# rnpnr/ogl_beamforming

Measured on AMD Instinct MI355X. Metric: beamformed voxels/s (and %HBM-roofline), 256-ch 3D DAS 512^3, 1/2/4/8 GPUs, higher is better.
Workload: dtype f32

## Files before the change

### ogl_beamforming_amd/csrc/bf_kernels.h

```cpp
#ifndef BF_KERNELS_H
#define BF_KERNELS_H

#include <stdint.h>
#include <hip/hip_runtime_api.h>

static const int bf_kind_byte_size[6]     = {2, 4, 4, 8, 2, 4};
static const int bf_kind_element_size[6]  = {2, 2, 4, 4, 2, 2};
static const int bf_kind_element_count[6] = {1, 2, 1, 2, 1, 2};
static const int bf_kind_complex[6]       = {0, 1, 0, 1, 0, 1};
enum { BF_BASE_I16 = 0, BF_BASE_F32 = 1, BF_BASE_F16 = 2 };
static const int bf_kind_base[6] = {BF_BASE_I16, BF_BASE_I16, BF_BASE_F32, BF_BASE_F32, BF_BASE_F16, BF_BASE_F16};

typedef struct {
	float    sin_a, cos_a;
	float    focus_x, focus_z;
	uint32_t flags;
	float    pad[3];
} BfTransmit;
enum {
	BF_TX_ROWS    = 1u << 0,
	BF_RX_ROWS    = 1u << 1,
	BF_TX_NONE    = 1u << 2,
	BF_TX_PLANE   = 1u << 3,
	BF_RX_COLUMNS = 1u << 4,
};

enum { BF_DAS_RCA = 0, BF_DAS_HERCULES = 1, BF_DAS_FORCES = 2, BF_DAS_READI = 3 };

typedef struct {
	float xdc_transform[16];
	float voxel_transform[16];
	float pitch[2];
	const void       *rf;
	void             *out;
	const BfTransmit *transmits;
	const int16_t    *sparse_elements;
	const uint16_t   *readi_hadamard;
	unsigned long long *pair_counter;
	uint32_t *tile_counters;
	int32_t  family, interpolation, complex_data, coherency_weighting;
	int32_t  acquisition_count, channel_count, sample_count, sparse;
	float    sampling_frequency, inv_sampling_frequency, demodulation_frequency;
	float    inv_speed_of_sound, time_offset, f_number;
	float    speed_of_sound;
	float    turns_per_sample;
	float    first_transmit_weight;
	uint32_t size[3];
	uint32_t z_first, z_count;
	uint32_t readi_group_count, readi_group;
	uint32_t tile_shift[3];
	uint32_t split_shift;
	uint32_t blocks[3];
	uint32_t depth_major;
	uint32_t band_rows;
	uint32_t zero_offset;
	uint32_t tile_window_shift;
	float    edge_margin;
	uint32_t row_ends;
} BfDasArgs;

#define BF_STAGED_PAIRED_GROUP_MAX 60u

typedef struct {
	uint32_t u_axis;
	uint32_t u_shift, v_shift;
	uint32_t threads;
	uint32_t channel_chunk;
	uint32_t lds_bytes;
	uint32_t tiles[3];
	uint32_t depth_major;
	uint32_t walk_columns;
	uint32_t window_shift;
	uint32_t zero_offset;
	uint32_t uniform;
	uint32_t window_samples;
	uint32_t table_stride;
	void    *tables;
	uint32_t *violations;
} BfSeparableArgs;

typedef struct {
	float   *table;
	float   *extremes;
	uint32_t table_pitch;
	uint32_t inner_count, outer_count;
	uint32_t inner_coord;
	uint32_t inner_is_transmit;
	uint32_t tiles[3];
	uint32_t rows;
	uint32_t depth_major;
	uint32_t band_rows;
	uint32_t zero_offset;
	float    unit_scale2, samples_per_unit;
	void    *pairs;
	uint32_t phase_local;
} BfHerculesArgs;

typedef struct {
	const void *raw; void *out;
	const int16_t *channel_mapping;
	uint64_t in_row_bytes, out_row_bytes;
	uint32_t channels;
	int32_t  a1s2, base;
	uint32_t a1s2_scalars;
} BfIngestArgs;

typedef struct {
	const void *left, *right; void *out;
	uint32_t size[3];
	int64_t  in_stride[3], out_stride[3];
	int32_t  in_kind, out_kind, interleave;
} BfReshapeArgs;

typedef struct {
	const void *in; void *out;
	const float *hadamard_t;
	const float *hadamard_base;
	uint32_t     hadamard_base_order;
	uint32_t transmit_count, channel_count, sample_count;
	int64_t  out_stride[3];
	int32_t  in_kind, out_kind;
} BfDecodeArgs;

typedef struct {
	const void *in; void *out;
	const float *coefficients;
	const float *phasors;
	uint32_t filter_length, decimation, sample_count, batch_sample_count;
	int32_t  complex_filter, demodulate;
	float    sampling_frequency, demodulation_frequency;
	int64_t  in_stride[3], out_stride[3];
	int64_t  in_elements;
	uint32_t channels, transmits;
	int32_t  in_kind, out_kind;
} BfFilterArgs;

static inline uint32_t bf_walk_columns(uint32_t tiles_u) { return tiles_u % 4u == 0 ? 4u : (tiles_u % 2u == 0 ? 2u : 1u); }
#ifdef __HIPCC__
static __device__ __forceinline__ void bf_column_walk(uint32_t tile, uint32_t tiles_u, uint32_t tiles_z, uint32_t g, uint32_t &tu, uint32_t &tv, uint32_t &zl)
{
	const uint32_t r = tile / g, col = r / tiles_z, per_row = tiles_u / g;
	zl = r % tiles_z;
	tu = (col % per_row) * g + tile % g;
	tv = col / per_row;
// ... 58 lines not shown
```

### ogl_beamforming_amd/csrc/das_select.cpp

```cpp
#include "das_select.h"
#include "host_math.h"
#include "../../include/ogl_beamformer_lib.h"
#include <cmath>
#include <cstdio>
#include <cstdlib>
#include <cstring>

namespace bf {

const char *das_path_name(int path)
{
	static const char *names[] = {"general kernel", "separable-delay gather kernel", "separable-delay LDS-staged kernel", "per-voxel factored kernel",
	                              "HERCULES aligned-grid kernel", "per-voxel factored kernel with block-wide LDS staging",
	                              "?", "none: the frame is cleared"};
	return path >= 0 && path <= 7 ? names[path] : "?";
}

const char *das_kernel_name(int path)
{
	static const char *names[] = {"das_kernel", "das_rca_separable_kernel", "das_rca_staged_kernel", "das_factored_kernel",
	                              "das_hercules_kernel", "das_tile_kernel", "?", "(none)"};
	return path >= 0 && path <= 7 ? names[path] : "?";
}

// ... 242 lines not shown
	q.tiles[0] = (nu + (1u << best_u) - 1) >> best_u;
	q.tiles[1] = (nv + (1u << best_v) - 1) >> best_v;
	q.tiles[2] = zcount;
	q.walk_columns = 1u;
	return true;
}

static bool plan_staged(const BfDasArgs &a, const std::vector<BfTransmit> &tx, const float *xdc, const float *vox,
                        uint32_t zcount, BfSeparableArgs &q, bool allow_uniform = true)
{
	const Hooks &hk = hooks();
	const bool cplx = a.complex_data != 0;
	const bool cubic = a.interpolation == 2;
	if (a.interpolation != 1 && !(cubic && cplx)) return false;
	const uint32_t C = (uint32_t)a.channel_count, A = (uint32_t)a.acquisition_count;
	if ((uint64_t)C * A * (uint64_t)a.sample_count * (cplx ? 8u : 4u) >= (1ull << 31)) return false;
	const uint32_t A4 = (A + 3u) & ~3u;
	const int u_axis = (int)q.u_axis, v_axis = 1 - u_axis;
	const int r = (tx[0].flags & BF_RX_ROWS) ? 1 : 0, w = (tx[0].flags & BF_TX_ROWS) ? 1 : 0;
	float m[16];
	m4_mul(xdc, vox, m);
	const float samples_per_metre = a.sampling_frequency * a.inv_speed_of_sound;
	float step_u = std::fabs(m[4 * u_axis + r]) / (float)(a.size[u_axis] > 1 ? a.size[u_axis] - 1 : 1) * samples_per_metre;
	float step_v = std::fabs(vox[4 * v_axis + w]) / (float)(a.size[v_axis] > 1 ? a.size[v_axis] - 1 : 1) * samples_per_metre;
	bool all_plane = true; float max_sin = 0.f;
	for (const BfTransmit &t : tx) {
		all_plane &= (t.flags & BF_TX_PLANE) != 0;
		max_sin = std::fmax(max_sin, std::fabs(t.sin_a));
	}
	if (tx[0].flags & BF_TX_NONE) step_v = 0.f;
	else if (all_plane)           step_v *= max_sin;

	const uint32_t lds_cu = 160u * 1024u;
	uint32_t best_waves = 0, best_score = 0;
	BfSeparableArgs best = q;
	for (uint32_t threads_shift = 10; threads_shift >= 9; threads_shift--) {
		for (uint32_t vs = 4; vs <= 6; vs++) {
			if (vs + 4 > threads_shift) continue;
			uint32_t us = threads_shift - vs;
			if (us > 6) continue;
			if ((u_axis == 0 ? us : vs) < 4) continue;
			float spread = step_u * (float)((1u << us) - 1) + step_v * (float)((1u << vs) - 1);
			if (!(spread >= 0.f && spread <= 60.f)) continue;
			uint32_t need = (uint32_t)std::ceil(spread * 1.001f) + (cubic ? 6 : 4);
			uint32_t ws = need <= 32 ? 5 : need <= 64 ? 6 : 0;
			if (!ws) continue;
			if (hk.staged_shape_set) {
				const unsigned fu = (unsigned)hk.staged_shape[0], fv = (unsigned)hk.staged_shape[1], fw = (unsigned)hk.staged_shape[2];
				if (fu != us || fv != vs) continue;
				if (fw < ws || fw > 6) continue;
				ws = fw;
			}
			const bool uniform = allow_uniform && cplx && !cubic && u_axis == 0 && threads_shift == 10 && us == 6 && vs == 4 &&
			                     !hk.staged_nouniform;
			const uint32_t window = 1u << ws;
			if (((uint64_t)A4 << ws) > ((uint64_t)(cplx ? 4 : 8) << threads_shift)) continue;
			const uint64_t stage_elements = (uint64_t)A4 * window;
			for (uint32_t chunk = 8; chunk <= 64; chunk *= 2) {
				uint32_t cc = chunk < C ? chunk : C;
				uint64_t lds = cubic ? 12ull * ((uint64_t)A4 << vs) + 16ull * ((uint64_t)cc << us) + 32ull * (stage_elements + 3) + 4ull * (A4 + cc + 1) + 128
				             : cplx ? (uniform ? 0ull : 12ull * ((uint64_t)A4 << vs)) + 16ull * ((uint64_t)cc << us) + 16ull * (stage_elements + 3) + 4ull * (A4 + cc + 1) + 128
				                    :  4ull * ((uint64_t)A4 << vs) +  8ull * ((uint64_t)cc << us) +  8ull * (stage_elements + 4) + 4ull * (A4 + cc + 1) + 128;
				lds = (lds + 15) & ~15ull;
				if (lds > lds_cu) continue;
				uint32_t blocks = (uint32_t)(lds_cu / lds), by_waves = (cubic ? 1024u : 2048u) >> threads_shift;
				if (blocks > by_waves) blocks = by_waves;
				uint32_t waves = blocks << (threads_shift - 6);
				uint32_t balance = us > vs ? us - vs : vs - us;
				uint32_t score = (blocks >= 2 ? 1000u : 0u) + (cc << 2) + (8 - balance) + (window == 32 ? 500u : 0u) +
				                 (uniform && window == 32 ? 2000u : 0u);
				if (waves > best_waves || (waves == best_waves && score > best_score)) {
					best_waves = waves; best_score = score;
					best.u_shift = us; best.v_shift = vs; best.threads = 1u << threads_shift;
					best.channel_chunk = cc; best.lds_bytes = (uint32_t)lds; best.window_shift = ws; best.window_samples = window;
					best.uniform = uniform ? 1u : 0u;
					best.table_stride = uniform ? 4u * A4 + 16u + 16u * (A4 / 4u) * 48u : 0u;
				}
				if (cc == C) break;
			}
		}
	}
	if (best_waves && allow_uniform && cplx && !cubic && !hk.staged_nouniform && best.threads == 1024 && best.u_shift == 5 && best.v_shift == 5 &&
	    best.window_samples == 32) {
		const uint32_t ngroups = (A4 + BF_STAGED_PAIRED_GROUP_MAX - 1u) / BF_STAGED_PAIRED_GROUP_MAX;
		const uint64_t group = ((A4 + ngroups - 1u) / ngroups + 3u) & ~3u;
		const uint32_t cc = best.channel_chunk;
		uint64_t lds = 16ull * (group * 64 + 3) + 16ull * ((uint64_t)((cc + 1) & ~1u) << 5) + 4ull * (A4 + cc + 1) + 128;
		lds = (lds + 15) & ~15ull;
		if (ngroups <= 2 && lds <= lds_cu / 2 && ((cc & 1u) == 0 || cc == C)) {
			best.uniform = 2u;
			best.lds_bytes = (uint32_t)lds;
			best.table_stride = 4u * A4 + 16u + 16u * (A4 / 2u) * 48u;
		}
	}
	if (hk.staged_checked) best.depth_major |= 2u;
	if (best.uniform && (best.depth_major & 1u)) best.depth_major |= 4u;
	if (hk.debug)
		std::fprintf(stderr, "[beamformer] staged plan: step_u %.3f step_v %.3f waves %u u %u v %u w %u chunk %u lds %u uniform %u\n",
		             step_u, step_v, best_waves, best.u_shift, best.v_shift, best.window_samples, best.channel_chunk, best.lds_bytes, best.uniform);
	if (!best_waves) return false;
	q = best;
	uint32_t nu = a.size[u_axis], nv = a.size[v_axis];
	q.tiles[0] = (nu + (1u << q.u_shift) - 1) >> q.u_shift;
	q.tiles[1] = (nv + (1u << q.v_shift) - 1) >> q.v_shift;
	q.tiles[2] = zcount;
	q.walk_columns = bf_walk_columns(q.tiles[0]);
	return true;
}

static const uint32_t kHerculesRows = 8u;

static bool plan_hercules(const BfDasArgs &a, const std::vector<BfTransmit> &tx, const float *xdc, const float *vox,
                          uint32_t zcount, bool forced, BfHerculesArgs &q)
{
	if (a.family != BF_DAS_HERCULES || tx.empty()) return false;
	if (!forced) {
		if (a.size[0] < 32 || a.split_shift) return false;
		if (((a.size[0] + 63u) & ~63u) > a.size[0] + a.size[0] / 3u) return false;
	}
	auto W = [&](int row, int col) { return vox[4 * col + row]; };
	auto X = [&](int row, int col) { return xdc[4 * col + row]; };
	auto moves = [&](int row, int col) {
		if (a.size[col] <= 1) return false;
		for (int k = 0; k < 3; k++) if (X(row, k) != 0.f && W(k, col) != 0.f) return true;
		return false;
	};
	int inner = -1;
	for (int coord = 0; coord < 2 && inner < 0; coord++)
		if (!moves(coord, 0) && !moves(coord, 2)) inner = coord;
	if (inner == 0 && !moves(1, 0) && !moves(1, 2) && !moves(0, 1) && moves(1, 1)) inner = 1;
	if (inner < 0) return false;
	const bool rx_cols = (tx[0].flags & BF_RX_COLUMNS) != 0;
	const int  tx_coord = rx_cols ? 1 : 0;
	const uint32_t A = (uint32_t)a.acquisition_count, C = (uint32_t)a.channel_count;
	const uint32_t transmits = A - (a.sparse ? 1u : 0u);
	if (!transmits || !C) return false;
	q.inner_coord       = (uint32_t)inner;
	q.inner_is_transmit = inner == tx_coord;
	q.inner_count       = q.inner_is_transmit ? transmits : C;
	q.outer_count       = q.inner_is_transmit ? C : transmits;
	q.table_pitch       = (q.inner_count + 8u + 3u) & ~3u;
	q.tiles[0] = (a.size[0] + 63u) / 64u;
	q.rows     = kHerculesRows;
	q.tiles[1] = (a.size[1] + q.rows - 1u) / q.rows;
	q.tiles[2] = zcount;
	{
		float m[16];
		m4_mul(xdc, vox, m);
		const uint32_t ext[3] = {a.size[0], a.size[1], zcount};
		int depth = 2; float best = -1.f;
		for (int i = 0; i < 3; i++) {
			if (ext[i] <= 1) continue;
			float step = std::fabs(m[4 * i + 2]) / (float)(a.size[i] > 1 ? a.size[i] - 1 : 1);
			if (step > best) { best = step; depth = i; }
		}
		q.depth_major = tile_walk(depth, zcount, q.tiles[1], q.band_rows);
	}
	{
		static float cached_fs = 0.f, cached_c = 0.f, cached_s2 = 1.f, cached_k = 0.f;
		if (cached_fs != a.sampling_frequency || cached_c != a.speed_of_sound) {
			const double k_exact = (double)a.sampling_frequency / (double)a.speed_of_sound;
			double best = 1e9;
			for (int i = -4096; i <= 4096; i++) {
				uint32_t bits = 0x3F800000u + (uint32_t)i;
				float s2; std::memcpy(&s2, &bits, sizeof s2);
				double s  = std::sqrt((double)s2);
				float  kk = (float)(k_exact / s);
				double err = std::fabs((double)kk * s / k_exact - 1.0);
				if (err < best) { best = err; cached_s2 = s2; cached_k = kk; }
			}
			cached_fs = a.sampling_frequency; cached_c = a.speed_of_sound;
		}
// ... 417 lines not shown
```

### ogl_beamforming_amd/csrc/das_staged.hip

```cpp
#include "das_common.h"

typedef int i32x2 __attribute__((ext_vector_type(2)));
typedef __attribute__((address_space(3))) f32x2 lds_f32x2;
typedef __attribute__((address_space(3))) f32x4 lds_f32x4;
typedef float f32x3 __attribute__((ext_vector_type(3)));
typedef __attribute__((address_space(3))) f32x3 lds_f32x3;

__device__ __forceinline__ float staged_phase_turns(float k, float index)
{
	float p = k * index;
	float e = __builtin_fmaf(k, index, -p);
	return hw_fract(p) + e;
}

__device__ __forceinline__ bool staged_tile_of(const BfSeparableArgs &q, bool global_tables, uint32_t &tu, uint32_t &tv, uint32_t &zl)
{
	const bool paired = global_tables && (q.depth_major & 4u);
	const uint32_t zchunks = (q.tiles[2] + 31u) >> 5;
	const uint32_t total = paired ? q.tiles[0] * q.tiles[1] * zchunks * 32u : q.tiles[0] * q.tiles[1] * q.tiles[2];
	const uint32_t per   = (total + 7u) / 8u;
	const uint32_t tile  = (blockIdx.x & 7u) * per + (blockIdx.x >> 3);
	if (tile >= total) return false;
	if (paired) {
		uint32_t r = tile >> 5;
// ... 253 lines not shown
				else return 0.f;
			};
			auto batches = [&](auto checked) {
				constexpr bool CHECK = decltype(checked)::value;
				uint32_t lane_id = tid;
				asm volatile("" : "+v"(lane_id));
				const uint32_t lane_v = u_axis == 0 ? lane_id >> q.u_shift : lane_id & (V - 1);
				uint32_t tcs_at = tcs_base + (lane_v << 4), tz_at = tz_base + (lane_v << 3);
				uint32_t m_bits = 0x4B000002u;
				[[maybe_unused]] bool window_left = false;
				const f32x2 rr = {r_rel, r_rel};
				const_f32x4 *uni_row = nullptr;
				if constexpr (UNI)
					uni_row = (const_f32x4 *)(uintptr_t)(tile_tab + 4u * (uint32_t)A4 + 16u +
					                                      (size_t)__builtin_amdgcn_readfirstlane((int)(tid >> 6)) * (size_t)(A4 / 4) * 48u);
				for (int a = 0; a < A4; a += 4, m_bits += 4u * W) {
					uint32_t at[4]; f32x4 tap[4];
					const float M = __builtin_bit_cast(float, m_bits);
					const f32x2 M2 = {M, M};
					f32x4 cs01, cs23; f32x2 tz01, tz23;
					if constexpr (UNI) {
						const f32x4 tz = uni_row[0];
						cs01 = uni_row[1]; cs23 = uni_row[2];
						tz01 = f32x2{tz.x, tz.y}; tz23 = f32x2{tz.z, tz.w};
						uni_row += 3;
					} else {
						cs01 = *(lds_f32x4 *)(uintptr_t)tcs_at;
						cs23 = *(lds_f32x4 *)(uintptr_t)(tcs_at + V * 16u);
						tz01 = *(lds_f32x2 *)(uintptr_t)tz_at;
						tz23 = *(lds_f32x2 *)(uintptr_t)(tz_at + V * 8u);
						tcs_at += 2u * V * 16u; tz_at += 2u * V * 8u;
					}
					const f32x2 p01 = rr + tz01, p23 = rr + tz23;
					const f32x2 y01 = p01 + M2,  y23 = p23 + M2;
					const float ys[4] = {y01.x, y01.y, y23.x, y23.y};
					#pragma unroll
					for (int k = 0; k < 4; k++) {
						const uint32_t yb = __builtin_bit_cast(uint32_t, ys[k]);
						asm("v_lshlrev_b16 %0, 4, %1" : "=v"(at[k]) : "v"(yb));
						if constexpr (CHECK) {
							uint32_t k_abs = (uint32_t)((int)(yb - m_bits) + rfloor[cl] + tfl[a + k]);
							at[k] = k_abs < ulast ? at[k] + (uint32_t)k * W * 16u : (stage_elements + 2u) * 16u;
							window_left |= __builtin_amdgcn_ballot_w64((yb - m_bits) > W - 2u) != 0ull;
						}
					}
					#pragma unroll
					for (int k = 0; k < 4; k++) tap[k] = *(lds_f32x4 *)(uintptr_t)(at[k] + (CHECK ? 0u : (uint32_t)k * W * 16u));
					const float q0 = term(f32x2{cs01.x, cs01.y}, p01.x, tap[0]);
					const float q1 = term(f32x2{cs01.z, cs01.w}, p01.y, tap[1]);
					const float q2 = term(f32x2{cs23.x, cs23.y}, p23.x, tap[2]);
					const float q3 = term(f32x2{cs23.z, cs23.w}, p23.y, tap[3]);
					if constexpr (CW) { mag2 += f32x2{q0, q1}; mag2 += f32x2{q2, q3}; }
				}
				if constexpr (CHECK) { if (window_left) staged_violation_raise(); }
			};
			if (wave_safe) batches(std::false_type{});
			else           batches(std::true_type{});
			float sum_x = acc1.x - acc2.y, sum_y = acc1.y + acc2.x;
			asm volatile("" : "+v"(sum_x), "+v"(sum_y));
			const f32x4 r = *(volatile lds_f32x4 *)(uintptr_t)((uint32_t)(uintptr_t)(lds_f32x4 *)Rl + (uint32_t)cl * U * 16u);
			coherent.x = __builtin_fmaf(sum_x, r.y, __builtin_fmaf(-sum_y, r.z, coherent.x));
			coherent.y = __builtin_fmaf(sum_x, r.z, __builtin_fmaf(sum_y, r.y, coherent.y));
			if constexpr (CW) incoherent = __builtin_fmaf(__builtin_fabsf(r.w), mag2.x + mag2.y, incoherent);
		}
	}
	if (q.depth_major & 2u) staged_violation_report(tid);
	if (!inside) return;

	uint32_t x, y, lane_u_unused, thread = tid;
	asm volatile("" : "+v"(thread));
	voxel_of(thread, x, y, lane_u_unused);
	uint64_t out_index = (uint64_t)p.size[0] * p.size[1] * zl + (uint64_t)p.size[0] * y + x;
	if constexpr (CW) coherent = coherent * (coherent / incoherent);
	reinterpret_cast<f32x2 *>(p.out)[out_index] = coherent;
}

template <bool CW, int NL>
__device__ __forceinline__ void staged_paired_body(const BfDasArgs &p, const BfSeparableArgs &q)
{
	extern __shared__ __attribute__((aligned(16))) f32x4 staged_lds[];
	constexpr uint32_t U = 32, W = 32, B = 2 * W;
	const int C = p.channel_count, A = p.acquisition_count, S = p.sample_count;
	const uint32_t A4 = ((uint32_t)A + 3u) & ~3u;
	const uint32_t ngroups = (A4 + BF_STAGED_PAIRED_GROUP_MAX - 1u) / BF_STAGED_PAIRED_GROUP_MAX;
	const uint32_t G0 = ((A4 + ngroups - 1u) / ngroups + 3u) & ~3u;
	const int chunk = (int)q.channel_chunk;
	f32x4 *stage  = staged_lds + 2;
	f32x4 *R      = stage + (size_t)G0 * B + 1;
	int   *tfl    = reinterpret_cast<int *>(R + (size_t)((chunk + 1) & ~1) * U);
	int   *rfloor = tfl + A4;

	uint32_t tu, tv, zl;
	if (!staged_tile_of(q, true, tu, tv, zl)) return;
	const uint32_t z = p.z_first + zl;
	const uint32_t u_axis = q.u_axis, v_axis = 1u - q.u_axis;
	const bool rx_rows = (p.transmits[0].flags & BF_RX_ROWS) != 0;
	const uint32_t tid = threadIdx.x;
	if (q.depth_major & 2u) staged_violation_clear(tid);
	auto opaque_tid = [&]() -> uint32_t { uint32_t t = tid; asm volatile("" : "+v"(t)); return t; };

	const unsigned char *tile_tab = reinterpret_cast<const unsigned char *>(q.tables) + (size_t)(zl * q.tiles[1] + tv) * q.table_stride;
	typedef __attribute__((address_space(4))) const int const_int;
	const_int *tab_floor = (const_int *)(uintptr_t)tile_tab;
	for (uint32_t a = tid; a < A4; a += 1024u) tfl[a] = reinterpret_cast<const int *>(tile_tab)[a];
	if (tid == 0) stage[(size_t)G0 * B] = f32x4{0.f, 0.f, 0.f, 0.f};
	f32x2 range = *reinterpret_cast<const f32x2 *>(tile_tab + 4u * A4);
	{
		const float lo = range.x, hi = range.y;
		range.x = __builtin_bit_cast(float, __builtin_amdgcn_readfirstlane(__builtin_bit_cast(int, lo)));
		range.y = __builtin_bit_cast(float, __builtin_amdgcn_readfirstlane(__builtin_bit_cast(int, hi)));
	}

	const uint32_t wave = (uint32_t)__builtin_amdgcn_readfirstlane((int)(tid >> 6));
	const uint32_t h = (tid >> 5) & 1u, lu = tid & 31u;
	bool inside;
	{
		const uint32_t gu = tu * U + lu, gv = tv * 32u + wave;
		inside = gu < p.size[u_axis] && gv < p.size[v_axis];
	}
	const bool wave_inside = __builtin_amdgcn_ballot_w64(inside) != 0ull;

	const __amdgpu_buffer_rsrc_t rf_rsrc = __builtin_amdgcn_make_buffer_rsrc(
		const_cast<void *>(p.rf), 0, (int)((uint32_t)C * (uint32_t)A * (uint32_t)S * 8u), 0x00020000);
	auto lane_at_of = [&](int c0, int cl) -> uint32_t {
		return c0 + cl < C ? ((uint32_t)(c0 + cl) * (uint32_t)A * (uint32_t)S + (uint32_t)(rfloor[cl] + (int)(opaque_tid() & 31u))) * 8u : 0x80000000u;
	};
	auto stage_load = [&](uint32_t lane_at, uint32_t g, f32x2 (&regs)[NL]) {
		const uint32_t a0 = g * G0, gn = A4 - a0 < G0 ? A4 - a0 : G0;
		#pragma unroll
		for (int n = 0; n < NL; n++) {
			const uint32_t al = wave + (uint32_t)n * 16u, a = a0 + al;
			const bool real = al < gn && a < (uint32_t)A;
			const uint32_t off = real ? lane_at + ((a * (uint32_t)S + (uint32_t)tab_floor[real ? a : 0]) * 8u) : 0x80000000u;
			i32x2 v = __builtin_amdgcn_raw_buffer_load_b64(rf_rsrc, (int)off, 0, 0);
			regs[n] = __builtin_bit_cast(f32x2, v);
		}
	};
	auto stage_store = [&](uint32_t g, const f32x2 (&regs)[NL]) {
		const uint32_t a0 = g * G0, gn = A4 - a0 < G0 ? A4 - a0 : G0;
		const uint32_t tid = opaque_tid();
		const float half_minus_j = 0.5f - (float)(tid & 63u);
		#pragma unroll
		for (int n = 0; n < NL; n++) {
			const float sx = regs[n].x, sy = regs[n].y;
			const float nx = __builtin_bit_cast(float, __builtin_amdgcn_update_dpp(0, __builtin_bit_cast(int, sx), 0x130, 0xf, 0xf, true));
			const float ny = __builtin_bit_cast(float, __builtin_amdgcn_update_dpp(0, __builtin_bit_cast(int, sy), 0x130, 0xf, 0xf, true));
			const float dx = nx - sx, dy = ny - sy;
			const uint32_t e = tid + (uint32_t)n * 1024u;
			if (e < gn * B) stage[e] = f32x4{__builtin_fmaf(half_minus_j, dx, sx), __builtin_fmaf(half_minus_j, dy, sy), dx, dy};
		}
	};

	f32x2 coherent   = {0.f, 0.f};
	float incoherent = 0.f;
	auto exchange = [](float x, float y) -> float {
		const auto r = __builtin_amdgcn_permlane32_swap(__builtin_bit_cast(uint32_t, x), __builtin_bit_cast(uint32_t, y), false, false);
		return __builtin_bit_cast(float, (uint32_t)r[0]) + __builtin_bit_cast(float, (uint32_t)r[1]);
	};
	const f32x4 *Rl = R + (size_t)h * U + lu;
	const uint32_t ulast = (uint32_t)(S - 1);
	const const_f32x4 *rows = (const_f32x4 *)(uintptr_t)(tile_tab + 4u * A4 + 16u) + (size_t)wave * (A4 / 2u) * 3u;

	typedef __attribute__((address_space(4))) const BfDasArgs const_args;
	const_args *kernel_args = (const_args *)__builtin_amdgcn_kernarg_segment_ptr();
	for (int c0 = 0; c0 < C; c0 += chunk) {
		const int cn = (C - c0) < chunk ? (C - c0) : chunk;
		const int cn2 = (cn + 1) & ~1;
		__syncthreads();
		{
		const_args *ka = kernel_args;
		asm volatile("" : "+s"(ka));
		const uint32_t k_size[3] = {ka->size[0], ka->size[1], ka->size[2]};
		const float k_denom_u = fmaxf(1.0f, (float)k_size[u_axis] - 1.0f);
		const float k_pz = (float)z / fmaxf(1.0f, (float)k_size[2] - 1.0f);
		const float k_fs = ka->sampling_frequency, k_inv_c = ka->inv_speed_of_sound, k_c = ka->speed_of_sound, k_fnum = ka->f_number;
		const float k_phase = ka->demodulation_frequency * ka->inv_sampling_frequency;
		const float k_pitch = rx_rows ? ka->pitch[1] : ka->pitch[0];
		for (uint32_t e = opaque_tid(); e < (uint32_t)cn2 * U; e += 1024u) {
			uint32_t cl = e >> 5, iu = e & (U - 1);
			f32x4 entry = {0.f, 0.f, 0.f, 0.f};
			if ((int)cl < cn) {
				uint32_t c = (uint32_t)c0 + cl;
				float coord[3] = {0.f, 0.f, k_pz};
				coord[u_axis] = (float)(tu * U + iu) / k_denom_u;
				float wx, wy, wz, xx, xy, xz;
				m4_point(ka->voxel_transform, coord[0], coord[1], coord[2], wx, wy, wz);
				m4_point(ka->xdc_transform, wx, wy, wz, xx, xy, xz);
				float lateral = rx_rows ? xy : xx;
				float dx      = lateral - (float)c * k_pitch;
				float a_arg   = __builtin_fabsf(dx * (k_fnum * hw_rcp(__builtin_fabsf(xz))));
				float r_idx = div_speed_of_sound(hw_sqrt(dx * dx + xz * xz), k_inv_c, k_c) * k_fs;
				entry.x = r_idx;
				if (a_arg < 0.5f) {
					float cs    = hw_cos_turns(0.5f * a_arg);
					float apod  = cs * cs;
					float turns = staged_phase_turns(k_phase, r_idx);
					entry.y = apod * hw_cos_turns(turns);
					entry.z = apod * hw_sin_turns(turns);
					entry.w = apod;
				}
			}
			R[e] = entry;
		}
		}
		__syncthreads();
		for (uint32_t cl = opaque_tid(); cl < (uint32_t)cn2; cl += 1024u) {
			const float *row = reinterpret_cast<const float *>(R + (size_t)cl * U);
			float m = row[0];
			#pragma unroll 4
			for (uint32_t iu = 1; iu < U; iu++) m = fminf(m, row[4 * iu]);
			rfloor[cl] = (int)__builtin_floorf(m);
		}
		__syncthreads();
		for (uint32_t e = opaque_tid(); e < (uint32_t)cn2 * U; e += 1024u) {
			f32x4 entry = R[e];
			const uint32_t cl = e >> 5;
			const bool lane_safe = (int)cl >= cn || ((entry.x + range.x >= 0.f) && (entry.x + range.y < (float)(S - 1)));
			entry.x = (entry.x - (float)rfloor[cl]) + (float)((cl & 1u) * W);
			if (!lane_safe) entry.w = -entry.w;
			R[e] = entry;
		}
		__syncthreads();

		f32x2 regs[NL];
		stage_load(lane_at_of(c0, (int)h), 0, regs);
		for (int k = 0; k < cn2 / 2; k++) {
			f32x2 acc1a = {0.f, 0.f}, acc2a = {0.f, 0.f}, acc1b = {0.f, 0.f}, acc2b = {0.f, 0.f};
			f32x2 mag2 = {0.f, 0.f};
			for (uint32_t g = 0; g < ngroups; g++) {
				__syncthreads();
				stage_store(g, regs);
				__syncthreads();
				if (g + 1 < ngroups)     stage_load(lane_at_of(c0, 2 * k + (int)h), g + 1, regs);
				else if (2 * k + 2 < cn2) stage_load(lane_at_of(c0, 2 * k + 2 + (int)h), 0, regs);
				if (!wave_inside) continue;

				float r_rel, r_w;
				{
					const f32x4 r = Rl[(size_t)(2 * k) * U];
					r_rel = r.x; r_w = r.w;
				}
				if (__builtin_amdgcn_ballot_w64(r_w != 0.f) == 0) continue;
				const bool wave_safe = !(q.depth_major & 2u) && __builtin_amdgcn_ballot_w64(__builtin_signbitf(r_w)) == 0;
				auto term = [&](f32x2 cs, float pos, f32x4 tap, f32x2 &acc1, f32x2 &acc2) -> float {
					f32x2 sv = f32x2{tap.x, tap.y} + pos * f32x2{tap.z, tap.w};
					acc1 += sv.x * cs;
					acc2 += sv.y * cs;
					if constexpr (CW) return hw_sqrt(__builtin_fmaf(sv.y, sv.y, sv.x * sv.x));
					else return 0.f;
				};
				const uint32_t a0 = g * G0, gn = A4 - a0 < G0 ? A4 - a0 : G0;
				auto batches = [&](auto checked) {
					constexpr bool CHECK = decltype(checked)::value;
					uint32_t m_bits = 0x4B000002u;
					[[maybe_unused]] bool window_left = false;
					[[maybe_unused]] int rfl_h = 0;
					if constexpr (CHECK) rfl_h = rfloor[2 * k + (int)h] - (int)(h * W);
					const f32x2 rr = {r_rel, r_rel};
					const_f32x4 *row = rows + (size_t)(a0 / 2u) * 3u;
					for (uint32_t a = 0; a < gn; a += 2, m_bits += 2u * B) {
						uint32_t at[4]; f32x4 tap[4];
						const float M = __builtin_bit_cast(float, m_bits);
						const f32x2 M2 = {M, M};
						const f32x4 tz = row[0], cs0 = row[1], cs1 = row[2];
						row += 3;
						const f32x2 p0 = rr + f32x2{tz.x, tz.y}, p1 = rr + f32x2{tz.z, tz.w};
						const f32x2 y0 = p0 + M2, y1 = p1 + M2;
						const float ys[4] = {y0.x, y0.y, y1.x, y1.y};
						#pragma unroll
						for (int t = 0; t < 4; t++) {
							const uint32_t yb = __builtin_bit_cast(uint32_t, ys[t]);
							asm("v_lshlrev_b16 %0, 4, %1" : "=v"(at[t]) : "v"(yb));
							if constexpr (CHECK) {
								uint32_t lane_id = tid;
								asm volatile("" : "+v"(lane_id));
								const uint32_t rel = yb - m_bits;
								const uint32_t k_abs = (uint32_t)((int)rel + rfl_h + tfl[a0 + a + (uint32_t)(t >> 1)]);
								at[t] = k_abs < ulast ? at[t] + (uint32_t)(t >> 1) * B * 16u : (G0 * B + 2u) * 16u;
								window_left |= __builtin_amdgcn_ballot_w64(inside && rel - (lane_id & 32u) > W - 2u) != 0ull;
							}
						}
						#pragma unroll
						for (int t = 0; t < 4; t++) tap[t] = *(lds_f32x4 *)(uintptr_t)(at[t] + (CHECK ? 0u : (uint32_t)(t >> 1) * B * 16u));
						const float qa0 = term(f32x2{cs0.x, cs0.y}, p0.x, tap[0], acc1a, acc2a);
						const float qb0 = term(f32x2{cs0.z, cs0.w}, p0.y, tap[1], acc1b, acc2b);
						const float qa1 = term(f32x2{cs1.x, cs1.y}, p1.x, tap[2], acc1a, acc2a);
						const float qb1 = term(f32x2{cs1.z, cs1.w}, p1.y, tap[3], acc1b, acc2b);
						if constexpr (CW) { mag2 += f32x2{qa0, qb0}; mag2 += f32x2{qa1, qb1}; }
					}
					if constexpr (CHECK) { if (window_left) staged_violation_raise(); }
				};
				if (wave_safe) batches(std::false_type{});
				else           batches(std::true_type{});
				if (g + 1 < ngroups) continue;
				float sa_x = acc1a.x - acc2a.y, sa_y = acc1a.y + acc2a.x;
				float sb_x = acc1b.x - acc2b.y, sb_y = acc1b.y + acc2b.x;
				asm volatile("" : "+v"(sa_x), "+v"(sa_y), "+v"(sb_x), "+v"(sb_y));
				const f32x4 r = *(volatile lds_f32x4 *)(uintptr_t)((uint32_t)(uintptr_t)(lds_f32x4 *)Rl + (uint32_t)(2 * k) * U * 16u);
				const float ca_x = __builtin_fmaf(sa_x, r.y, -sa_y * r.z), ca_y = __builtin_fmaf(sa_x, r.z, sa_y * r.y);
				const float cb_x = __builtin_fmaf(sb_x, r.y, -sb_y * r.z), cb_y = __builtin_fmaf(sb_x, r.z, sb_y * r.y);
				coherent.x += exchange(ca_x, cb_x);
				coherent.y += exchange(ca_y, cb_y);
				if constexpr (CW) incoherent += exchange(__builtin_fabsf(r.w) * mag2.x, __builtin_fabsf(r.w) * mag2.y);
			}
		}
	}
	if (q.depth_major & 2u) staged_violation_report(tid);
	uint32_t thread = tid;
	asm volatile("" : "+v"(thread));
	const uint32_t gu = tu * U + (thread & 31u), gv = tv * 32u + (thread >> 6) + ((thread >> 5) & 1u) * 16u;
	if (!(gu < p.size[u_axis] && gv < p.size[v_axis])) return;
	const uint32_t x = u_axis == 0 ? gu : gv, y = u_axis == 0 ? gv : gu;
	uint64_t out_index = (uint64_t)p.size[0] * p.size[1] * zl + (uint64_t)p.size[0] * y + x;
	if constexpr (CW) coherent = coherent * (coherent / incoherent);
	reinterpret_cast<f32x2 *>(p.out)[out_index] = coherent;
}

template <bool CW, int VS, int WS, int NL, bool UNI, bool PAIRED>
__global__ __launch_bounds__(1024, 8) void das_rca_staged_kernel(const BfDasArgs p, const BfSeparableArgs q)
{
	if constexpr (PAIRED) staged_paired_body<CW, NL>(p, q);
	else                  staged_body<CW, VS, WS, NL, UNI>(p, q);
}

template <bool CW, int VS, int WS, int NL, bool UNI>
static hipError_t launch_staged(const BfDasArgs *a, const BfSeparableArgs *q, hipStream_t s)
{
	uint32_t total = q->tiles[0] * q->tiles[1] * q->tiles[2];
	if (UNI && (q->depth_major & 4u)) total = q->tiles[0] * q->tiles[1] * ((q->tiles[2] + 31u) >> 5) * 32u;
	uint32_t grid  = ((total + 7u) / 8u) * 8u;
	auto kernel = das_rca_staged_kernel<CW, VS, WS, NL, UNI, false>;
	hipError_t e = hipFuncSetAttribute((const void *)kernel, hipFuncAttributeMaxDynamicSharedMemorySize, (int)q->lds_bytes);
	if (e != hipSuccess) return e;
	hipLaunchKernelGGL(kernel, dim3(grid), dim3(q->threads), q->lds_bytes, s, *a, *q);
	return hipGetLastError();
}

template <bool CW, int VS, int WS, bool UNI>
static hipError_t launch_staged_loads(const BfDasArgs *a, const BfSeparableArgs *q, hipStream_t s)
{
	const uint32_t A4 = ((uint32_t)a->acquisition_count + 3u) & ~3u;
	const uint32_t passes = ((A4 << WS) + q->threads - 1) / q->threads;
	switch (passes) {
	case 1: return launch_staged<CW, VS, WS, 1, UNI>(a, q, s);
	case 2: return launch_staged<CW, VS, WS, 2, UNI>(a, q, s);
	case 3: return launch_staged<CW, VS, WS, 3, UNI>(a, q, s);
	case 4: return launch_staged<CW, VS, WS, 4, UNI>(a, q, s);
	}
	return hipErrorInvalidValue;
}

template <bool CW, int NL>
static hipError_t launch_staged_paired(const BfDasArgs *a, const BfSeparableArgs *q, hipStream_t s)
{
	const uint32_t total = q->tiles[0] * q->tiles[1] * ((q->depth_major & 4u) ? ((q->tiles[2] + 31u) >> 5) * 32u : q->tiles[2]);
	const uint32_t grid  = ((total + 7u) / 8u) * 8u;
	auto kernel = das_rca_staged_kernel<CW, 5, 5, NL, true, true>;
	hipError_t e = hipFuncSetAttribute((const void *)kernel, hipFuncAttributeMaxDynamicSharedMemorySize, (int)q->lds_bytes);
	if (e != hipSuccess) return e;
	hipLaunchKernelGGL(kernel, dim3(grid), dim3(1024), q->lds_bytes, s, *a, *q);
	return hipGetLastError();
}

template <bool CW>
static hipError_t launch_staged_shape(const BfDasArgs *a, const BfSeparableArgs *q, hipStream_t s)
{
	if (q->uniform == 2) {
		if (q->u_shift != 5 || q->v_shift != 5 || q->window_samples != 32 || q->threads != 1024 || !q->tables ||
		    ((q->channel_chunk & 1u) && (int)q->channel_chunk < a->channel_count)) return hipErrorInvalidValue;
		const uint32_t A4 = ((uint32_t)a->acquisition_count + 3u) & ~3u;
		const uint32_t ngroups = (A4 + BF_STAGED_PAIRED_GROUP_MAX - 1u) / BF_STAGED_PAIRED_GROUP_MAX;
		const uint32_t G0 = ((A4 + ngroups - 1u) / ngroups + 3u) & ~3u;
		switch ((G0 * 64u + 1023u) / 1024u) {
		case 1:
		case 2: return launch_staged_paired<CW, 2>(a, q, s);
		case 3: return launch_staged_paired<CW, 3>(a, q, s);
		case 4: return launch_staged_paired<CW, 4>(a, q, s);
		}
		return hipErrorInvalidValue;
	}
	if (q->uniform) {
		if (q->u_axis != 0 || q->u_shift != 6 || q->v_shift != 4 || q->threads != 1024 || !q->tables) return hipErrorInvalidValue;
		if (q->window_samples == 32) return launch_staged_loads<CW, 4, 5, true>(a, q, s);
		if (q->window_samples == 64) return launch_staged_loads<CW, 4, 6, true>(a, q, s);
		return hipErrorInvalidValue;
	}
	switch ((q->v_shift << 4) | q->window_shift) {
	case (4 << 4) | 5: return launch_staged_loads<CW, 4, 5, false>(a, q, s);
	case (5 << 4) | 5: return launch_staged_loads<CW, 5, 5, false>(a, q, s);
	case (6 << 4) | 5: return launch_staged_loads<CW, 6, 5, false>(a, q, s);
	case (4 << 4) | 6: return launch_staged_loads<CW, 4, 6, false>(a, q, s);
	case (5 << 4) | 6: return launch_staged_loads<CW, 5, 6, false>(a, q, s);
	case (6 << 4) | 6: return launch_staged_loads<CW, 6, 6, false>(a, q, s);
	}
	return hipErrorInvalidValue;
}

extern "C" hipError_t bf_launch_das_staged(const BfDasArgs *a, const BfSeparableArgs *q, hipStream_t s)
{
	if (!a->complex_data || a->interpolation != BF_INTERP_LINEAR) return hipErrorInvalidValue;
	if ((uint64_t)a->channel_count * (uint64_t)a->acquisition_count * (uint64_t)a->sample_count * 8u >= (1ull << 31)) return hipErrorInvalidValue;
	return a->coherency_weighting ? launch_staged_shape<true>(a, q, s) : launch_staged_shape<false>(a, q, s);
}

template <int VS>
__global__ __launch_bounds__(256) void staged_tables_kernel(const BfDasArgs p, const BfSeparableArgs q)
{
	extern __shared__ __attribute__((aligned(16))) f32x4 tables_lds[];
	constexpr uint32_t V = 1u << VS;
	const int A = p.acquisition_count;
	const int A4 = (A + 3) & ~3;
	float *t  = reinterpret_cast<float *>(tables_lds);
	f32x2 *cs = reinterpret_cast<f32x2 *>(t + (size_t)A4 * V);
	f32x2 *wave_range = cs + (size_t)A4 * V;
	const uint32_t tv = blockIdx.x % q.tiles[1], zl = blockIdx.x / q.tiles[1];
	const uint32_t z  = p.z_first + zl;
	const uint32_t v_axis = 1u - q.u_axis;
	const float denom[3] = {fmaxf(1.0f, (float)p.size[0] - 1.0f), fmaxf(1.0f, (float)p.size[1] - 1.0f),
	                        fmaxf(1.0f, (float)p.size[2] - 1.0f)};
	const float pz = (float)z / denom[2];
	const float phase_k = p.demodulation_frequency * p.inv_sampling_frequency;
	const uint32_t tid = threadIdx.x, nthreads = blockDim.x;
	for (uint32_t e = tid; e < (uint32_t)A4 * V; e += nthreads) {
		uint32_t a = e >> VS, iv = e & (V - 1);
		float cs_c = 0.f, cs_s = 0.f, t_idx = 0.f;
		if (a < (uint32_t)A) {
			float coord[3] = {0.f, 0.f, pz};
			coord[v_axis] = (float)(tv * V + iv) / denom[v_axis];
			float wx, wy, wz;
			m4_point(p.voxel_transform, coord[0], coord[1], coord[2], wx, wy, wz);
			const BfTransmit t_a = p.transmits[a];
			float dist = 0.f;
			if (!(t_a.flags & BF_TX_NONE)) {
				float px = (t_a.flags & BF_TX_ROWS) ? wy : wx;
				if (t_a.flags & BF_TX_PLANE) dist = px * t_a.sin_a + wz * t_a.cos_a;
				else { float ddx = px - t_a.focus_x, ddz = wz - t_a.focus_z; dist = hw_sqrt(ddx * ddx + ddz * ddz); }
			}
			t_idx = (div_speed_of_sound(dist, p) + p.time_offset) * p.sampling_frequency;
			float turns = staged_phase_turns(phase_k, t_idx);
			cs_c = hw_cos_turns(turns); cs_s = hw_sin_turns(turns);
		}
		t[e] = t_idx; cs[e] = f32x2{cs_c, cs_s};
	}
	__syncthreads();
	{
		float lo = __builtin_inff(), hi = -__builtin_inff();
		for (uint32_t e = tid; e < (uint32_t)A * V; e += nthreads) { lo = fminf(lo, t[e]); hi = fmaxf(hi, t[e]); }
		for (int off = 32; off > 0; off >>= 1) {
			lo = fminf(lo, __shfl_xor(lo, off, 64));
			hi = fmaxf(hi, __shfl_xor(hi, off, 64));
		}
		if ((tid & 63u) == 0) wave_range[tid >> 6] = f32x2{lo, hi};
	}
	__syncthreads();
	unsigned char *tile_tab = reinterpret_cast<unsigned char *>(q.tables) + (size_t)blockIdx.x * q.table_stride;
	if (tid == 0) {
		f32x2 range = wave_range[0];
// ... 61 lines not shown
```

Measured before the change: 173.0 million.

## Rebalance paired staged-kernel group split and precompute per-channel RF base offsets

New measurement: 176.2 million, median of 6. +1.9%, better.

```diff
diff --git a/ogl_beamforming_amd/csrc/bf_kernels.h b/ogl_beamforming_amd/csrc/bf_kernels.h
--- a/ogl_beamforming_amd/csrc/bf_kernels.h
+++ b/ogl_beamforming_amd/csrc/bf_kernels.h
@@ -60,6 +60,37 @@
 } BfDasArgs;
 
 #define BF_STAGED_PAIRED_GROUP_MAX 60u
+#define BF_STAGED_PAIRED_LDS_BUDGET (80u * 1024u)
+
+#ifdef __HIPCC__
+#define BF_HOST_DEVICE __host__ __device__
+#else
+#define BF_HOST_DEVICE
+#endif
+static inline BF_HOST_DEVICE uint32_t bf_staged_paired_lds_bytes(uint32_t group, uint32_t channel_chunk, uint32_t a4)
+{
+	const uint32_t lds = 16u * (group * 64u + 3u) + 16u * (((channel_chunk + 1u) & ~1u) << 5) + 4u * (a4 + 2u * (channel_chunk + 2u)) + 128u;
+	return (lds + 15u) & ~15u;
+}
+static inline BF_HOST_DEVICE uint32_t bf_staged_paired_passes(uint32_t group)
+{
+	const uint32_t passes = (group + 15u) / 16u;
+	return passes < 2u ? 2u : passes;
+}
+static inline BF_HOST_DEVICE bool bf_staged_paired_split(uint32_t a4, uint32_t channel_chunk, uint32_t *g0, uint32_t *g1)
+{
+	uint32_t gmax = BF_STAGED_PAIRED_GROUP_MAX;
+	while (gmax >= 4u && bf_staged_paired_lds_bytes(gmax, channel_chunk, a4) > BF_STAGED_PAIRED_LDS_BUDGET) gmax -= 4u;
+	*g0 = *g1 = 0u;
+	if (a4 < 4u || (a4 & 3u) || gmax < 4u || a4 > 2u * gmax) return false;
+	if (a4 <= gmax) { *g0 = a4; return true; }
+	uint32_t best_key = ~0u;
+	for (uint32_t first = gmax; 2u * first >= a4; first -= 4u) {
+		const uint32_t key = (bf_staged_paired_passes(first) + bf_staged_paired_passes(a4 - first)) * 256u + ((first & 15u) ? 128u : 0u) + first;
+		if (key < best_key) { best_key = key; *g0 = first; *g1 = a4 - first; }
+	}
+	return true;
+}
 
 typedef struct {
 	uint32_t u_axis;
diff --git a/ogl_beamforming_amd/csrc/das_select.cpp b/ogl_beamforming_amd/csrc/das_select.cpp
--- a/ogl_beamforming_amd/csrc/das_select.cpp
+++ b/ogl_beamforming_amd/csrc/das_select.cpp
@@ -348,12 +348,10 @@
 	}
 	if (best_waves && allow_uniform && cplx && !cubic && !hk.staged_nouniform && best.threads == 1024 && best.u_shift == 5 && best.v_shift == 5 &&
 	    best.window_samples == 32) {
-		const uint32_t ngroups = (A4 + BF_STAGED_PAIRED_GROUP_MAX - 1u) / BF_STAGED_PAIRED_GROUP_MAX;
-		const uint64_t group = ((A4 + ngroups - 1u) / ngroups + 3u) & ~3u;
 		const uint32_t cc = best.channel_chunk;
-		uint64_t lds = 16ull * (group * 64 + 3) + 16ull * ((uint64_t)((cc + 1) & ~1u) << 5) + 4ull * (A4 + cc + 1) + 128;
-		lds = (lds + 15) & ~15ull;
-		if (ngroups <= 2 && lds <= lds_cu / 2 && ((cc & 1u) == 0 || cc == C)) {
+		uint32_t g0, g1;
+		if (bf_staged_paired_split(A4, cc, &g0, &g1) && ((cc & 1u) == 0 || cc == C)) {
+			const uint64_t lds = bf_staged_paired_lds_bytes(g0, cc, A4);
 			best.uniform = 2u;
 			best.lds_bytes = (uint32_t)lds;
 			best.table_stride = 4u * A4 + 16u + 16u * (A4 / 2u) * 48u;
diff --git a/ogl_beamforming_amd/csrc/das_staged.hip b/ogl_beamforming_amd/csrc/das_staged.hip
--- a/ogl_beamforming_amd/csrc/das_staged.hip
+++ b/ogl_beamforming_amd/csrc/das_staged.hip
@@ -359,13 +359,15 @@
 	constexpr uint32_t U = 32, W = 32, B = 2 * W;
 	const int C = p.channel_count, A = p.acquisition_count, S = p.sample_count;
 	const uint32_t A4 = ((uint32_t)A + 3u) & ~3u;
-	const uint32_t ngroups = (A4 + BF_STAGED_PAIRED_GROUP_MAX - 1u) / BF_STAGED_PAIRED_GROUP_MAX;
-	const uint32_t G0 = ((A4 + ngroups - 1u) / ngroups + 3u) & ~3u;
 	const int chunk = (int)q.channel_chunk;
+	uint32_t G0, G1;
+	if (!bf_staged_paired_split(A4, q.channel_chunk, &G0, &G1)) return;
+	const uint32_t ngroups = G1 ? 2u : 1u;
 	f32x4 *stage  = staged_lds + 2;
 	f32x4 *R      = stage + (size_t)G0 * B + 1;
 	int   *tfl    = reinterpret_cast<int *>(R + (size_t)((chunk + 1) & ~1) * U);
 	int   *rfloor = tfl + A4;
+	uint32_t *rbase = reinterpret_cast<uint32_t *>(rfloor + ((chunk + 2) & ~1));
 
 	uint32_t tu, tv, zl;
 	if (!staged_tile_of(q, true, tu, tv, zl)) return;
@@ -399,32 +401,36 @@
 
 	const __amdgpu_buffer_rsrc_t rf_rsrc = __builtin_amdgcn_make_buffer_rsrc(
 		const_cast<void *>(p.rf), 0, (int)((uint32_t)C * (uint32_t)A * (uint32_t)S * 8u), 0x00020000);
-	auto lane_at_of = [&](int c0, int cl) -> uint32_t {
-		return c0 + cl < C ? ((uint32_t)(c0 + cl) * (uint32_t)A * (uint32_t)S + (uint32_t)(rfloor[cl] + (int)(opaque_tid() & 31u))) * 8u : 0x80000000u;
-	};
+	auto lane_at_of = [&](int cl) -> uint32_t { return rbase[cl] + ((opaque_tid() & 31u) << 3); };
 	auto stage_load = [&](uint32_t lane_at, uint32_t g, f32x2 (&regs)[NL]) {
-		const uint32_t a0 = g * G0, gn = A4 - a0 < G0 ? A4 - a0 : G0;
+		const uint32_t a0 = g ? G0 : 0u, gn = g ? G1 : G0;
+		int fl[NL];
+		#pragma unroll
+		for (int n = 0; n < NL; n++) {
+			const uint32_t a = a0 + wave + (uint32_t)n * 16u;
+			fl[n] = tab_floor[a < A4 ? a : A4 - 1u];
+		}
 		#pragma unroll
 		for (int n = 0; n < NL; n++) {
 			const uint32_t al = wave + (uint32_t)n * 16u, a = a0 + al;
 			const bool real = al < gn && a < (uint32_t)A;
-			const uint32_t off = real ? lane_at + ((a * (uint32_t)S + (uint32_t)tab_floor[real ? a : 0]) * 8u) : 0x80000000u;
+			const uint32_t off = real ? lane_at + ((a * (uint32_t)S + (uint32_t)fl[n]) * 8u) : 0x80000000u;
 			i32x2 v = __builtin_amdgcn_raw_buffer_load_b64(rf_rsrc, (int)off, 0, 0);
 			regs[n] = __builtin_bit_cast(f32x2, v);
 		}
 	};
 	auto stage_store = [&](uint32_t g, const f32x2 (&regs)[NL]) {
-		const uint32_t a0 = g * G0, gn = A4 - a0 < G0 ? A4 - a0 : G0;
+		const uint32_t gn = g ? G1 : G0;
 		const uint32_t tid = opaque_tid();
 		const float half_minus_j = 0.5f - (float)(tid & 63u);
 		#pragma unroll
 		for (int n = 0; n < NL; n++) {
+			if (wave + (uint32_t)n * 16u >= gn) break;
 			const float sx = regs[n].x, sy = regs[n].y;
 			const float nx = __builtin_bit_cast(float, __builtin_amdgcn_update_dpp(0, __builtin_bit_cast(int, sx), 0x130, 0xf, 0xf, true));
 			const float ny = __builtin_bit_cast(float, __builtin_amdgcn_update_dpp(0, __builtin_bit_cast(int, sy), 0x130, 0xf, 0xf, true));
 			const float dx = nx - sx, dy = ny - sy;
-			const uint32_t e = tid + (uint32_t)n * 1024u;
-			if (e < gn * B) stage[e] = f32x4{__builtin_fmaf(half_minus_j, dx, sx), __builtin_fmaf(half_minus_j, dy, sy), dx, dy};
+			stage[tid + (uint32_t)n * 1024u] = f32x4{__builtin_fmaf(half_minus_j, dx, sx), __builtin_fmaf(half_minus_j, dy, sy), dx, dy};
 		}
 	};
 
@@ -486,7 +492,9 @@
 			float m = row[0];
 			#pragma unroll 4
 			for (uint32_t iu = 1; iu < U; iu++) m = fminf(m, row[4 * iu]);
-			rfloor[cl] = (int)__builtin_floorf(m);
+			const int fl = (int)__builtin_floorf(m);
+			rfloor[cl] = fl;
+			rbase[cl] = c0 + (int)cl < C ? ((uint32_t)(c0 + (int)cl) * (uint32_t)A * (uint32_t)S + (uint32_t)fl) * 8u : 0x80000000u;
 		}
 		__syncthreads();
 		for (uint32_t e = opaque_tid(); e < (uint32_t)cn2 * U; e += 1024u) {
@@ -500,25 +508,21 @@
 		__syncthreads();
 
 		f32x2 regs[NL];
-		stage_load(lane_at_of(c0, (int)h), 0, regs);
+		stage_load(lane_at_of((int)h), 0, regs);
 		for (int k = 0; k < cn2 / 2; k++) {
-			f32x2 acc1a = {0.f, 0.f}, acc2a = {0.f, 0.f}, acc1b = {0.f, 0.f}, acc2b = {0.f, 0.f};
-			f32x2 mag2 = {0.f, 0.f};
-			for (uint32_t g = 0; g < ngroups; g++) {
-				__syncthreads();
-				stage_store(g, regs);
-				__syncthreads();
-				if (g + 1 < ngroups)     stage_load(lane_at_of(c0, 2 * k + (int)h), g + 1, regs);
-				else if (2 * k + 2 < cn2) stage_load(lane_at_of(c0, 2 * k + 2 + (int)h), 0, regs);
-				if (!wave_inside) continue;
-
-				float r_rel, r_w;
-				{
-					const f32x4 r = Rl[(size_t)(2 * k) * U];
-					r_rel = r.x; r_w = r.w;
-				}
-				if (__builtin_amdgcn_ballot_w64(r_w != 0.f) == 0) continue;
-				const bool wave_safe = !(q.depth_major & 2u) && __builtin_amdgcn_ballot_w64(__builtin_signbitf(r_w)) == 0;
+			float r_rel = 0.f;
+			int mode = 0;
+			if (wave_inside) {
+				const f32x4 r = Rl[(size_t)(2 * k) * U];
+				r_rel = r.x;
+				if (__builtin_amdgcn_ballot_w64(r.w != 0.f) != 0)
+					mode = (!(q.depth_major & 2u) && __builtin_amdgcn_ballot_w64(__builtin_signbitf(r.w)) == 0) ? 1 : 2;
+			}
+			auto rounds = [&](auto mode_c) {
+				constexpr int MODE = decltype(mode_c)::value;
+				constexpr bool CHECK = MODE == 2;
+				f32x2 acc1a = {0.f, 0.f}, acc2a = {0.f, 0.f}, acc1b = {0.f, 0.f}, acc2b = {0.f, 0.f};
+				f32x2 mag2 = {0.f, 0.f};
 				auto term = [&](f32x2 cs, float pos, f32x4 tap, f32x2 &acc1, f32x2 &acc2) -> float {
 					f32x2 sv = f32x2{tap.x, tap.y} + pos * f32x2{tap.z, tap.w};
 					acc1 += sv.x * cs;
@@ -526,60 +530,68 @@
 					if constexpr (CW) return hw_sqrt(__builtin_fmaf(sv.y, sv.y, sv.x * sv.x));
 					else return 0.f;
 				};
-				const uint32_t a0 = g * G0, gn = A4 - a0 < G0 ? A4 - a0 : G0;
-				auto batches = [&](auto checked) {
-					constexpr bool CHECK = decltype(checked)::value;
-					uint32_t m_bits = 0x4B000002u;
-					[[maybe_unused]] bool window_left = false;
-					[[maybe_unused]] int rfl_h = 0;
-					if constexpr (CHECK) rfl_h = rfloor[2 * k + (int)h] - (int)(h * W);
-					const f32x2 rr = {r_rel, r_rel};
-					const_f32x4 *row = rows + (size_t)(a0 / 2u) * 3u;
-					for (uint32_t a = 0; a < gn; a += 2, m_bits += 2u * B) {
-						uint32_t at[4]; f32x4 tap[4];
-						const float M = __builtin_bit_cast(float, m_bits);
-						const f32x2 M2 = {M, M};
-						const f32x4 tz = row[0], cs0 = row[1], cs1 = row[2];
-						row += 3;
-						const f32x2 p0 = rr + f32x2{tz.x, tz.y}, p1 = rr + f32x2{tz.z, tz.w};
-						const f32x2 y0 = p0 + M2, y1 = p1 + M2;
-						const float ys[4] = {y0.x, y0.y, y1.x, y1.y};
-						#pragma unroll
-						for (int t = 0; t < 4; t++) {
-							const uint32_t yb = __builtin_bit_cast(uint32_t, ys[t]);
-							asm("v_lshlrev_b16 %0, 4, %1" : "=v"(at[t]) : "v"(yb));
-							if constexpr (CHECK) {
-								uint32_t lane_id = tid;
-								asm volatile("" : "+v"(lane_id));
-								const uint32_t rel = yb - m_bits;
-								const uint32_t k_abs = (uint32_t)((int)rel + rfl_h + tfl[a0 + a + (uint32_t)(t >> 1)]);
-								at[t] = k_abs < ulast ? at[t] + (uint32_t)(t >> 1) * B * 16u : (G0 * B + 2u) * 16u;
-								window_left |= __builtin_amdgcn_ballot_w64(inside && rel - (lane_id & 32u) > W - 2u) != 0ull;
+				for (uint32_t g = 0; g < ngroups; g++) {
+					__syncthreads();
+					stage_store(g, regs);
+					__syncthreads();
+					if (g + 1 < ngroups)     stage_load(lane_at_of(2 * k + (int)h), g + 1, regs);
+					else if (2 * k + 2 < cn2) stage_load(lane_at_of(2 * k + 2 + (int)h), 0, regs);
+					if constexpr (MODE != 0) {
+						const uint32_t a0 = g ? G0 : 0u, gn = g ? G1 : G0;
+						uint32_t m_bits = 0x4B000002u;
+						[[maybe_unused]] bool window_left = false;
+						[[maybe_unused]] int rfl_h = 0;
+						if constexpr (CHECK) rfl_h = rfloor[2 * k + (int)h] - (int)(h * W);
+						const f32x2 rr = {r_rel, r_rel};
+						const_f32x4 *row = rows + (size_t)(a0 / 2u) * 3u;
+						for (uint32_t a = 0; a < gn; a += 2, m_bits += 2u * B) {
+							uint32_t at[4]; f32x4 tap[4];
+							const float M = __builtin_bit_cast(float, m_bits);
+							const f32x2 M2 = {M, M};
+							const f32x4 tz = row[0], cs0 = row[1], cs1 = row[2];
+							row += 3;
+							const f32x2 p0 = rr + f32x2{tz.x, tz.y}, p1 = rr + f32x2{tz.z, tz.w};
+							const f32x2 y0 = p0 + M2, y1 = p1 + M2;
+							const float ys[4] = {y0.x, y0.y, y1.x, y1.y};
+							#pragma unroll
+							for (int t = 0; t < 4; t++) {
+								const uint32_t yb = __builtin_bit_cast(uint32_t, ys[t]);
+								asm("v_lshlrev_b16 %0, 4, %1" : "=v"(at[t]) : "v"(yb));
+								if constexpr (CHECK) {
+									uint32_t lane_id = tid;
+									asm volatile("" : "+v"(lane_id));
+									const uint32_t rel = yb - m_bits;
+									const uint32_t k_abs = (uint32_t)((int)rel + rfl_h + tfl[a0 + a + (uint32_t)(t >> 1)]);
+									at[t] = k_abs < ulast ? at[t] + (uint32_t)(t >> 1) * B * 16u : (G0 * B + 2u) * 16u;
+									window_left |= __builtin_amdgcn_ballot_w64(inside && rel - (lane_id & 32u) > W - 2u) != 0ull;
+								}
 							}
+							#pragma unroll
+							for (int t = 0; t < 4; t++) tap[t] = *(lds_f32x4 *)(uintptr_t)(at[t] + (CHECK ? 0u : (uint32_t)(t >> 1) * B * 16u));
+							const float qa0 = term(f32x2{cs0.x, cs0.y}, p0.x, tap[0], acc1a, acc2a);
+							const float qb0 = term(f32x2{cs0.z, cs0.w}, p0.y, tap[1], acc1b, acc2b);
+							const float qa1 = term(f32x2{cs1.x, cs1.y}, p1.x, tap[2], acc1a, acc2a);
+							const float qb1 = term(f32x2{cs1.z, cs1.w}, p1.y, tap[3], acc1b, acc2b);
+							if constexpr (CW) { mag2 += f32x2{qa0, qb0}; mag2 += f32x2{qa1, qb1}; }
 						}
-						#pragma unroll
-						for (int t = 0; t < 4; t++) tap[t] = *(lds_f32x4 *)(uintptr_t)(at[t] + (CHECK ? 0u : (uint32_t)(t >> 1) * B * 16u));
-						const float qa0 = term(f32x2{cs0.x, cs0.y}, p0.x, tap[0], acc1a, acc2a);
-						const float qb0 = term(f32x2{cs0.z, cs0.w}, p0.y, tap[1], acc1b, acc2b);
-						const float qa1 = term(f32x2{cs1.x, cs1.y}, p1.x, tap[2], acc1a, acc2a);
-						const float qb1 = term(f32x2{cs1.z, cs1.w}, p1.y, tap[3], acc1b, acc2b);
-						if constexpr (CW) { mag2 += f32x2{qa0, qb0}; mag2 += f32x2{qa1, qb1}; }
+						if constexpr (CHECK) { if (window_left) staged_violation_raise(); }
 					}
-					if constexpr (CHECK) { if (window_left) staged_violation_raise(); }
-				};
-				if (wave_safe) batches(std::false_type{});
-				else           batches(std::true_type{});
-				if (g + 1 < ngroups) continue;
-				float sa_x = acc1a.x - acc2a.y, sa_y = acc1a.y + acc2a.x;
-				float sb_x = acc1b.x - acc2b.y, sb_y = acc1b.y + acc2b.x;
-				asm volatile("" : "+v"(sa_x), "+v"(sa_y), "+v"(sb_x), "+v"(sb_y));
-				const f32x4 r = *(volatile lds_f32x4 *)(uintptr_t)((uint32_t)(uintptr_t)(lds_f32x4 *)Rl + (uint32_t)(2 * k) * U * 16u);
-				const float ca_x = __builtin_fmaf(sa_x, r.y, -sa_y * r.z), ca_y = __builtin_fmaf(sa_x, r.z, sa_y * r.y);
-				const float cb_x = __builtin_fmaf(sb_x, r.y, -sb_y * r.z), cb_y = __builtin_fmaf(sb_x, r.z, sb_y * r.y);
-				coherent.x += exchange(ca_x, cb_x);
-				coherent.y += exchange(ca_y, cb_y);
-				if constexpr (CW) incoherent += exchange(__builtin_fabsf(r.w) * mag2.x, __builtin_fabsf(r.w) * mag2.y);
-			}
+				}
+				if constexpr (MODE != 0) {
+					float sa_x = acc1a.x - acc2a.y, sa_y = acc1a.y + acc2a.x;
+					float sb_x = acc1b.x - acc2b.y, sb_y = acc1b.y + acc2b.x;
+					asm volatile("" : "+v"(sa_x), "+v"(sa_y), "+v"(sb_x), "+v"(sb_y));
+					const f32x4 r = *(volatile lds_f32x4 *)(uintptr_t)((uint32_t)(uintptr_t)(lds_f32x4 *)Rl + (uint32_t)(2 * k) * U * 16u);
+					const float ca_x = __builtin_fmaf(sa_x, r.y, -sa_y * r.z), ca_y = __builtin_fmaf(sa_x, r.z, sa_y * r.y);
+					const float cb_x = __builtin_fmaf(sb_x, r.y, -sb_y * r.z), cb_y = __builtin_fmaf(sb_x, r.z, sb_y * r.y);
+					coherent.x += exchange(ca_x, cb_x);
+					coherent.y += exchange(ca_y, cb_y);
+					if constexpr (CW) incoherent += exchange(__builtin_fabsf(r.w) * mag2.x, __builtin_fabsf(r.w) * mag2.y);
+				}
+			};
+			if (mode == 1)      rounds(std::integral_constant<int, 1>{});
+			else if (mode == 2) rounds(std::integral_constant<int, 2>{});
+			else                rounds(std::integral_constant<int, 0>{});
 		}
 	}
 	if (q.depth_major & 2u) staged_violation_report(tid);
@@ -646,10 +658,9 @@
 		if (q->u_shift != 5 || q->v_shift != 5 || q->window_samples != 32 || q->threads != 1024 || !q->tables ||
 		    ((q->channel_chunk & 1u) && (int)q->channel_chunk < a->channel_count)) return hipErrorInvalidValue;
 		const uint32_t A4 = ((uint32_t)a->acquisition_count + 3u) & ~3u;
-		const uint32_t ngroups = (A4 + BF_STAGED_PAIRED_GROUP_MAX - 1u) / BF_STAGED_PAIRED_GROUP_MAX;
-		const uint32_t G0 = ((A4 + ngroups - 1u) / ngroups + 3u) & ~3u;
-		switch ((G0 * 64u + 1023u) / 1024u) {
-		case 1:
+		uint32_t G0, G1;
+		if (!bf_staged_paired_split(A4, q->channel_chunk, &G0, &G1) || q->lds_bytes < bf_staged_paired_lds_bytes(G0, q->channel_chunk, A4)) return hipErrorInvalidValue;
+		switch (bf_staged_paired_passes(G0)) {
 		case 2: return launch_staged_paired<CW, 2>(a, q, s);
 		case 3: return launch_staged_paired<CW, 3>(a, q, s);
 		case 4: return launch_staged_paired<CW, 4>(a, q, s);
```
